# maniacs-ops/ringpop-go

Measured on AMD Instinct MI355X. Metric: simulated member-rounds/sec at 64k members, higher is better.
Workload: dtype u32; 1 GPU; config3_cascade: 65536 members, 655 killed at r=10; rounds 5-592 timed (steady state, kill, suspect wave; faulty wave from r>=35 in window); members=65536, live_member_rounds=38153303, parallelism=1 GPU

## Files before the change

### include/swimsim.h

```cpp
#ifndef SWIMSIM_H
#define SWIMSIM_H
#include <stddef.h>
#include <stdint.h>

#ifdef __cplusplus
extern "C" {
#endif

#define SWIMSIM_ABI_VERSION 16

enum {
    SWIMSIM_OK = 0,
    SWIMSIM_EINVAL = -1,
    SWIMSIM_ENOMEM = -2,
    SWIMSIM_EHIP = -3,
    SWIMSIM_ECAPACITY = -4,
    SWIMSIM_ERANGE = -5
};

enum { SWIMSIM_ALIVE = 0, SWIMSIM_SUSPECT = 1, SWIMSIM_FAULTY = 2, SWIMSIM_LEAVE = 3, SWIMSIM_TOMBSTONE = 4,
       SWIMSIM_UNKNOWN = 7 };
#define SWIMSIM_SOURCE_NONE (-1)

typedef struct swimsim_config {
    uint32_t num_members;
    uint32_t device;
    int64_t t0_ms;
    uint32_t protocol_period_ms;
    uint32_t suspect_timeout_ms;
    uint32_t faulty_timeout_ms;
    uint32_t tombstone_timeout_ms;
    uint32_t ping_request_size;
    uint32_t max_reverse_full_sync_jobs;
    uint32_t p_factor;
    uint64_t seed;
    const char *addresses;
    uint32_t addr_stride;
    uint32_t max_rounds;
    uint64_t message_pool_bytes;
    uint32_t observer_begin, observer_end;
    const struct swimsim_tuning *tuning;
} swimsim_config;

typedef struct swimsim_tuning {
    int32_t hot_slots;
    int32_t dense_slots;
    int32_t cs_async;
    int32_t cs_async_rows;
    int32_t cs_narrow_rows;
    int32_t cs_ref;
    int32_t fault_inject;
    int32_t defer_test;
    int32_t cs_defer;
    int32_t resp_echo;
} swimsim_tuning;

enum {
    SWIMSIM_EV_KILL = 1,
    SWIMSIM_EV_REVIVE = 2,
    SWIMSIM_EV_REINCARNATE = 3,
    SWIMSIM_EV_LEAVE = 4,
    SWIMSIM_EV_PARTITION = 5,
    SWIMSIM_EV_HEAL = 6,
    SWIMSIM_EV_REAP = 7,
    SWIMSIM_EV_CLOCK = 8
};
typedef struct swimsim_event { uint32_t round; uint32_t kind; int32_t a; int32_t b; } swimsim_event;

enum {
    SWIMSIM_C_ROUNDS, SWIMSIM_C_PINGS, SWIMSIM_C_PINGS_OK, SWIMSIM_C_PINGREQS, SWIMSIM_C_HELPER_CALLS,
    SWIMSIM_C_HELPER_ERRORS, SWIMSIM_C_INCONCLUSIVE, SWIMSIM_C_SUSPECT_DECL, SWIMSIM_C_APPLIED,
    SWIMSIM_C_REFUTES, SWIMSIM_C_FULL_SYNCS, SWIMSIM_C_FULL_SYNCS_PINGREQ, SWIMSIM_C_RFS_DONE,
    SWIMSIM_C_RFS_OMITTED, SWIMSIM_C_TIMERS_FIRED, SWIMSIM_C_MSG_CHANGES, SWIMSIM_C_HEAL_ATTEMPTS,
    SWIMSIM_C_HEAL_FAILURES, SWIMSIM_NCOUNTERS
};

typedef struct swimsim swimsim_t;
// ... 139 lines not shown
```

### ringpop-go_amd/csrc/swimsim_device.h

```cpp
#pragma once
#include <hip/hip_runtime.h>
#include <stdint.h>

namespace swimdev {

constexpr uint32_t ST_ALIVE = 0, ST_SUSPECT = 1, ST_FAULTY = 2, ST_LEAVE = 3, ST_TOMB = 4, ST_UNKNOWN = 7;
constexpr uint32_t SRC_NONE = 0xFFFFFFFFu;
constexpr uint32_t NO_DEADLINE = 0xFFFFFFFFu;
constexpr uint8_t DP_NONE = 0xFF;
constexpr uint32_t DE_NONE = 0xFFFFFFFFu;
__host__ __device__ inline uint32_t de_p(uint32_t x) { return x >> 24; }
__host__ __device__ inline uint32_t de_src(uint32_t x) { return (x & 0xFFFFFFu) == 0xFFFFFFu ? SRC_NONE : (x & 0xFFFFFFu); }
__host__ __device__ inline uint32_t de_x(uint32_t src, uint32_t p) { return (src & 0xFFFFFFu) | (p << 24); }

enum Counter {
    C_ROUNDS, C_PINGS, C_PINGS_OK, C_PINGREQS, C_HELPER_CALLS, C_HELPER_ERRORS, C_INCONCLUSIVE,
    C_SUSPECT_DECL, C_APPLIED, C_REFUTES, C_FULL_SYNCS, C_FULL_SYNCS_PINGREQ, C_RFS_DONE, C_RFS_OMITTED,
    C_TIMERS_FIRED, C_MSG_CHANGES, C_HEAL_ATTEMPTS, C_HEAL_FAILURES, C_NCOUNTERS,
    C_X_MERGED = C_NCOUNTERS, C_X_APPLIED, C_X_ISSUED, C_X_CS_ROWS, C_X_CS_DUP,
    C_X_MERGED_R, C_X_APPLIED_R, C_X_RISSUED, C_X_RCALLS, C_X_BUMPED, C_X_CS_ROWS_N, C_X_CSD_SCANNED,
    C_X_DENSE_RESP, C_X_DENSE_JOBS, C_X_JOBS_APPLIED, C_X_DENSE_HEAL,
    C_X_DEFER, C_X_DEFER_EQ, C_X_DEFER_NOROW, C_X_DEFER_REP, C_X_DEFER_UNDO,
    C_X_DEFER_REP_DIFF, C_X_DEFER_UNDO_DIFF, C_X_DEFER_FS, C_X_DEFER_UNDO_OVER, C_X_DEFER_CLEAN,
    C_X_ISSUE_SNAPS, C_X_LAZY_LATE, C_X_LAZY_MAT,
    C_X_ECHO, C_NALL
};

constexpr int CTR_SHARDS = 64, CTR_STRIDE = 64;
static_assert(C_NALL <= CTR_STRIDE, "counter block too small");
constexpr uint32_t POOL_SHARDS = 64, POOL_CUR_STRIDE = 16;

enum ErrBits : uint32_t {
    E_POOL = 1, E_DENSE = 2, E_ECAP = 4, E_SHORT = 8, E_ITER = 16, E_COUNT = 32, E_XCAP = 64
};

struct MsgDesc {
    uint32_t off_lo, off_hi;
    uint32_t len;
    uint32_t kind;
};

struct DS {
    uint32_t N, NP, NL, lo, NB, NBW;
    uint32_t W;
    uint32_t pfactor, K, maxjobs;
    uint32_t to_susp, to_faulty, to_tomb;
    uint32_t ecap;
    uint64_t seed;
// ... 42 lines not shown
    uint64_t wev_mask;
    uint4 **wevs;
    unsigned long long **wevts;
    uint32_t *wev_cnt;
    uint32_t wev_cap;
    unsigned long long *useq;
    uint32_t *hidx;
    uint32_t *hlist;
    uint32_t *hmw;
    uint2 *hde;
    uint32_t *colx;
    uint32_t *hotnew;
    uint32_t *hot_cnt;
    uint32_t HP;
    int32_t *nhe;
    uint32_t *ucl, *uhk, *ucold, *ucnt;
    uint2 *ulog;
    uint32_t *ulog_cnt;
    uint32_t ulog_cap;
    uint32_t ulog_stride;
    uint32_t defer_test;
    uint32_t *ilen;
    int32_t *ilast;
};
constexpr uint32_t ULOG_CAP = 1024, ULOG_STRIDE = ULOG_CAP + 256;
constexpr uint32_t SRC_PEND = 0x7FFFFFFEu, SRC_CLAIM = 0x7FFFFFFDu;
constexpr uint32_t DIRTY_CARRIED = 2u;

__device__ __forceinline__ uint32_t hot_slot(const DS &d, uint32_t m) { return d.hidx ? d.hidx[m] : SRC_NONE; }

__host__ __device__ inline bool is_pingable(uint32_t st) { return st <= ST_SUSPECT; }

__device__ __forceinline__ uint32_t clock_of(const DS &d, uint32_t o, uint32_t r) { return r + (uint32_t)d.coff[o]; }

constexpr uint32_t RT_LOOKUP = 0, RT_COLD = 8191, RT_MAXSLOTS = 8128;
__host__ __device__ inline uint32_t rec_m(const uint4 &r) { return r.x & 0xFFFFFFu; }
__host__ __device__ inline uint32_t rec_st(const uint4 &r) { return (r.x >> 24) & 7u; }
__host__ __device__ inline uint32_t rec_e(const uint4 &r) { return r.y & 0xFFFFFFu; }
__host__ __device__ inline uint32_t rec_tag(const uint4 &r) { return (r.x >> 27) | ((r.y >> 24) << 5); }
__host__ __device__ inline uint32_t tag_of_slot(uint32_t hk) { return hk == SRC_NONE ? RT_COLD : hk + 1u; }
__host__ __device__ inline uint4 rec_make(uint32_t m, uint32_t st, uint32_t e, uint32_t src, uint32_t sinc, uint32_t tag) {
    return make_uint4(m | (st << 24) | (tag << 27), e | ((tag >> 5) << 24), src, sinc);
}
__host__ __device__ inline uint4 rec_retag(const uint4 &r, uint32_t tag) {
    return make_uint4((r.x & 0x07FFFFFFu) | (tag << 27), (r.y & 0xFFFFFFu) | ((tag >> 5) << 24), r.z, r.w);
}
// ... 142 lines not shown
```

### ringpop-go_amd/csrc/swimsim_engine.hip

```cpp
#include "swimsim_kernels.hip"
#include "swimsim_xchg.hip"
#include "swimsim_census.hip"
#include "swimsim_route.hip"
#include "swimsim_forward.hip"
#include "swimsim_ringcs.hip"

#include <hipcub/hipcub.hpp>
#include <rccl/rccl.h>

#include <algorithm>
#include <cmath>
#include <condition_variable>
#include <cstdarg>
#include <cstdio>
#include <cstring>
#include <memory>
#include <mutex>
#include <string>
#include <thread>
#include <vector>

#include "../../include/swimsim.h"

using namespace swimdev;
// ... 340 lines not shown
    unsigned long long *rc_key = nullptr;
    uint32_t *rc_cnt = nullptr, *rc_rep = nullptr, *rc_dif = nullptr, *rc_hl = nullptr, *rc_csr = nullptr, *rc_out = nullptr;
    size_t rc_cap = 0;
    bool rc_lds = false;
    double rc_split[3] = {0, 0, 0};
    int32_t *fw_own = nullptr, *fw_handler = nullptr, *fw_holder = nullptr, *fw_next = nullptr;
    uint32_t *fw_ent = nullptr, *fw_key = nullptr, *fw_bins = nullptr;
    uint8_t *fw_outcome = nullptr, *fw_hops = nullptr;
    size_t fw_own_cap = 0, fw_req_cap = 0, fw_ent_cap = 0, fw_bins_cap = 0;
    double fw_split[3] = {0, 0, 0};
    int csr_mode = 1;
    CsrSet csr, csr2;
    size_t csr_sbw_words = 0;
    uint32_t csr_ecap = 4096, csr_rcap = 1024, csr_KP = 0;
    uint64_t csr_launches = 0;
    uint32_t csr_side_min = 4097;
    int fault_inject = 0;
    int defer_test = 0;
    int cs_defer = 1;
    uint32_t rounds_left = 0;
    uint32_t round_deferred = 0;
    bool cs_carried = false;
    int resp_echo = 1;
    bool cs_defer_log = false;
    uint64_t cs_skipped_rounds = 0, cs_carried_rows = 0, cs_forced = 0, cs_units_base[3] = {0, 0, 0};
    bool colx_stale = false;
    std::string err;

    int fail(int code, const char *fmt, ...) {
        char buf[512];
        va_list ap;
        va_start(ap, fmt);
        vsnprintf(buf, sizeof buf, fmt, ap);
        va_end(ap);
        err = buf;
        return code;
    }
};

#define HIPCHK(h, x)                                                                             \
    do {                                                                                         \
        hipError_t e_ = (x);                                                                     \
        if (e_ != hipSuccess) return (h)->fail(SWIMSIM_EHIP, "%s: %s", #x, hipGetErrorString(e_)); \
    } while (0)

namespace {
// ... 485 lines not shown
    if (st && nrows != ~0u && csr_side_wanted(h, n)) {
        if (h->csr2_used) HIPCHK(h, hipStreamWaitEvent(st, h->ev_csr2, 0));
        const int rc = csr_hash(h, h->csr2, list, cnt, n, st);
        HIPCHK(h, hipEventRecord(h->ev_csr2, st));
        h->csr2_used = true;
        if (rc <= 0) return rc;
    }
    Scope sc(h, kind == CS_WIDE ? F_CS_WIDE : F_CS_NARROW, st);
    launch_checksum_kind(h->d, list, cnt, n, kind, st ? st : h->s);
    return 0;
}

void hot_flush(swimsim *h, uint32_t ol0, uint32_t n) {
    if (!h->d.hidx || n == 0) return;
    hipLaunchKernelGGL(k_hot_flush, dim3(blocks_for_waves(n)), dim3(SWIM_WAVE_BLOCK), 0, h->s, h->d, ol0, n);
}

void hot_reset(swimsim *h, bool flush) {
    if (!h->d.hidx) return;
    if (flush) hot_flush(h, 0, h->NL);
    hipMemsetAsync(h->d.hidx, 0xFF, (size_t)h->N * 4, h->s);
    hipMemsetAsync(h->d.hotnew, 0, (size_t)h->d.NBIT * 4, h->s);
    hipMemsetAsync(h->d.hot_cnt, 0, 8, h->s);
    hipLaunchKernelGGL(k_nhe_reset, dim3(blocks_for_threads(h->NL)), dim3(256), 0, h->s, h->d);
}

void hot_update(swimsim *h) {
    if (!h->d.hidx) return;
    hipLaunchKernelGGL(k_hot_extend, dim3(1), dim3(1024), 0, h->s, h->d);
    hipLaunchKernelGGL(k_hot_fill, dim3(blocks_for_waves(h->NL)), dim3(SWIM_WAVE_BLOCK), 0, h->s, h->d);
}

int retire_half(swimsim *h, uint32_t g) {
    if (!h->side_pend[g]) return 0;
    HIPCHK(h, hipStreamWaitEvent(h->s, h->ev_side[g], 0));
    const uint32_t lo = h->d.dense_cap + g * h->snap_cap;
    hipLaunchKernelGGL(k_side_retire, dim3(blocks_for_threads(h->NL)), dim3(256), 0, h->s, h->d, lo, lo + h->snap_cap);
    h->side_pend[g] = false;
    h->side_pending = h->side_pend[0] || h->side_pend[1];
    return 0;
}

int sync_side(swimsim *h) {
    if (!h->side_pending) return 0;
    for (uint32_t g = 0; g < 2; g++)
        if (int rc = retire_half(h, (h->side_gen + g) % 2)) return rc;
// ... 704 lines not shown
        hipEventCreateWithFlags(&h->ev_side[0], hipEventDisableTiming) != hipSuccess ||
        hipEventCreateWithFlags(&h->ev_side[1], hipEventDisableTiming) != hipSuccess ||
        hipEventCreateWithFlags(&h->ev_rt, hipEventDisableTiming) != hipSuccess) {
        h->err = "hipStreamCreate / hipEventCreate failed";
        return bail(SWIMSIM_EHIP);
    }
    const swimsim_tuning *tun = cfg->tuning;
    if (tun && tun->cs_async >= 0) h->cs_async = tun->cs_async != 0;
    if (tun && tun->cs_narrow_rows >= 0) h->cs_narrow_rows = (uint32_t)tun->cs_narrow_rows;
    if (tun && tun->cs_ref >= 0) h->csr_mode = tun->cs_ref;
    if (tun && tun->fault_inject > 0) h->fault_inject = tun->fault_inject;
    if (tun && tun->defer_test > 0) h->defer_test = tun->defer_test;
    if (tun && tun->cs_defer >= 0) h->cs_defer = tun->cs_defer;
    if (const char *v = getenv("SWIMSIM_CS_DEFER")) h->cs_defer = atoi(v);
    if (const char *v = getenv("SWIMSIM_CS_DEFER_LOG")) h->cs_defer_log = atoi(v) != 0;
    if (h->cs_defer < 0 || h->cs_defer > 2) {
        h->err = "swimsim_tuning.cs_defer is -1, 0, 1 or 2";
        return bail(SWIMSIM_EINVAL);
    }
    if (tun && tun->resp_echo >= 0) h->resp_echo = tun->resp_echo;
    if (const char *v = getenv("SWIMSIM_RESP_ECHO")) h->resp_echo = atoi(v);
    if (h->resp_echo < 0 || h->resp_echo > 1) {
        h->err = "swimsim_tuning.resp_echo is -1, 0 or 1";
        return bail(SWIMSIM_EINVAL);
    }
    if (h->fault_inject & 32) h->csr_ecap = 24;
    if (h->fault_inject & 256) h->csr_side_min = 1024;
    if (const char *v = getenv("SWIMSIM_SYNC_SPIN")) h->sync_spin = atoi(v) != 0;
    if (const char *v = getenv("SWIMSIM_SIDE2"))
        if (atoi(v) == 0 && h->side2) { hipStreamDestroy(h->side2); h->side2 = nullptr; }
    DS &d = h->d;
    d.N = h->N; d.NP = h->NP; d.NL = h->NL; d.lo = h->lo;
    d.NB = h->NP / 64;
    d.NBW = (d.NB + 63) / 64;
    d.NBIT = ((h->NP / 32) + 3) & ~3u;
    d.W = h->W; d.pfactor = h->pfactor; d.K = h->K; d.maxjobs = h->maxjobs;
    d.to_susp = h->to_susp; d.to_faulty = h->to_faulty; d.to_tomb = h->to_tomb;
    d.seed = h->seed;
    const size_t rows = (size_t)h->NL * h->NP;
    int rc = 0;
    if ((rc = dalloc(h, &d.mw, rows, "member words")) || (rc = dalloc(h, &d.dent, rows, "dissemination entries")) ||
        (rc = dalloc(h, &d.tst, rows, "timer states")) ||
        (rc = dalloc(h, &d.tmr, rows, "timers")) ||
        (rc = dalloc(h, &d.ping, h->NL, "ping")) || (rc = dalloc(h, &d.maxp, h->NL, "maxp")) ||
        (rc = dalloc(h, &d.dcnt, h->NL, "dcnt")) || (rc = dalloc(h, &d.dirty, h->NL, "dirty")) ||
        (rc = dalloc(h, &d.cs, h->NL, "cs")) || (rc = dalloc(h, &d.it_idx, h->NL, "it_idx")) ||
        (rc = dalloc(h, &d.it_ep, h->NL, "it_ep")) || (rc = dalloc(h, &d.tmin, h->NL, "tmin")) ||
        (rc = dalloc(h, &d.njobs, h->NL, "njobs")) || (rc = dalloc(h, &d.jobs, (size_t)h->NL * h->maxjobs, "jobs")) ||
        (rc = dalloc(h, &d.dbit, (size_t)h->NL * d.NBIT, "dbit")) || (rc = dalloc(h, &d.tblk, (size_t)h->NL * d.NB, "tblk")) ||
        (rc = dalloc(h, &d.live, h->N, "live")) || (rc = dalloc(h, &d.part, h->N, "part")) ||
        (rc = dalloc(h, &d.coff, h->N, "clock offsets")) ||
        (rc = dalloc(h, &d.ctr, (size_t)CTR_SHARDS * CTR_STRIDE, "counters")) || (rc = dalloc(h, &d.err, 4, "err")) ||
        (rc = dalloc(h, &d.clen, h->NL, "clen")) || (rc = dalloc(h, &d.clast, h->NL, "clast")) ||
        (rc = dalloc(h, &d.cpslot, h->NL, "cpslot")) || (rc = dalloc(h, &d.nhe, h->NL, "cold entry counts")) ||
        (rc = dalloc(h, &d.colx, d.NBIT, "divergent columns")) || (rc = dalloc(h, &d.ucl, h->N, "divergent column list")) ||
        (rc = dalloc(h, &d.uhk, h->N, "divergent column hot slots")) || (rc = dalloc(h, &d.ucold, h->N, "cold divergent columns")) ||
        (rc = dalloc(h, &d.ucnt, 2, "divergent column counts")))
        return bail(rc);
    hipMemset(d.nhe, 0, (size_t)h->NL * 4);
    hipMemset(d.coff, 0, (size_t)h->N * 4);
    h->coff.assign(h->N, 0);
    hipMemset(d.colx, 0xFF, (size_t)d.NBIT * 4);
    hipMemset(d.cpslot, 0xFF, (size_t)h->NL * 4);
    {
        uint32_t hp = std::min<uint32_t>(2048u, h->NP);
        if (tun && tun->hot_slots >= 0) hp = std::min<uint32_t>((uint32_t)tun->hot_slots, h->NP);
        hp = std::min<uint32_t>((hp + 63) & ~63u, RT_MAXSLOTS);
        d.hidx = nullptr; d.hlist = nullptr; d.hmw = nullptr; d.hde = nullptr; d.hotnew = nullptr; d.hot_cnt = nullptr;
        d.HP = 0;
        if (hp) {
            if ((rc = dalloc(h, &d.hidx, h->N, "hot index")) || (rc = dalloc(h, &d.hlist, hp, "hot list")) ||
                (rc = dalloc(h, &d.hmw, (size_t)h->NL * hp, "hot member words")) ||
                (rc = dalloc(h, &d.hde, (size_t)h->NL * hp, "hot dissemination cells")) ||
                (rc = dalloc(h, &d.hotnew, d.NBIT, "hot candidates")) || (rc = dalloc(h, &d.hot_cnt, 2, "hot count")))
                return bail(rc);
            d.HP = hp;
            hot_reset(h, false);
        }
    }
    {
        std::vector<uint32_t> aw((size_t)h->N * 6, 0u);
        for (uint32_t m = 0; m < h->N; m++) {
            uint8_t b[24] = {0};
            memcpy(b, h->addrs[m].data(), h->W);
            for (int w = 0; w < 6; w++)
                aw[(size_t)m * 6 + w] = (uint32_t)b[4 * w] | ((uint32_t)b[4 * w + 1] << 8) | ((uint32_t)b[4 * w + 2] << 16) |
                                        ((uint32_t)b[4 * w + 3] << 24);
        }
        uint32_t *dev = nullptr;
        if ((rc = dalloc(h, &dev, aw.size(), "address words"))) return bail(rc);
        if (hipMemcpy(dev, aw.data(), aw.size() * 4, hipMemcpyHostToDevice) != hipSuccess) return bail(SWIMSIM_EHIP);
        d.addrw = dev;
// ... 1071 lines not shown
            if (f == F_CSPREP) b = csdups * 8.0 * h->N;
            if (f == F_CSD_SCAN) b = delta(C_X_CSD_SCANNED) * 4.0 * h->N;
            if (f == F_ISSUE) b = issued * 32.0;
            if (f == F_RECV) b = merge_bytes + recv_issue_bytes;
            if (f == F_RESP) b = resp_bytes;
            if (f == F_JOBS_MERGE) b = delta(C_X_DENSE_JOBS) * 5.0 * h->N + delta(C_X_JOBS_APPLIED) * 23.0;
            alg_bytes[f] = b;
        }
    }
    if (n) *n = F_NFAM;
    return SWIMSIM_OK;
}

int swimsim_kernel_units(swimsim_t *h, const char **names, double *values, size_t cap, size_t *n) {
    if (!h) return SWIMSIM_EINVAL;
    uint64_t c[CTR_STRIDE];
    if (int rc = read_counters(h, c)) return rc;
    static const char *kn[] = {"cs_rows_wide", "cs_rows_narrow", "cs_dup_rows", "recv_merged", "recv_applied",
                               "recv_issued", "recv_calls", "resp_merged", "resp_applied", "resp_bumped", "issued",
                               "bitmap_words_per_row", "hot_slots", "dense_resp", "dense_jobs", "jobs_applied",
                               "dense_heal", "defer", "defer_eq", "defer_norow", "defer_rep", "defer_undo",
                               "defer_rep_diff", "defer_undo_diff", "defer_fs", "defer_undo_over", "defer_clean",
                               "issue_snaps", "lazy_late", "lazy_mat", "resp_echoed",
                               "cs_skipped_rounds", "cs_carried_rows", "cs_forced"};
    const int ki[] = {C_X_CS_ROWS, C_X_CS_ROWS_N, C_X_CS_DUP, C_X_MERGED, C_X_APPLIED, C_X_RISSUED, C_X_RCALLS,
                      C_X_MERGED_R, C_X_APPLIED_R, C_X_BUMPED, C_X_ISSUED, -1, -2, C_X_DENSE_RESP, C_X_DENSE_JOBS,
                      C_X_JOBS_APPLIED, C_X_DENSE_HEAL, C_X_DEFER, C_X_DEFER_EQ, C_X_DEFER_NOROW, C_X_DEFER_REP,
                      C_X_DEFER_UNDO, C_X_DEFER_REP_DIFF, C_X_DEFER_UNDO_DIFF, C_X_DEFER_FS, C_X_DEFER_UNDO_OVER,
                      C_X_DEFER_CLEAN, C_X_ISSUE_SNAPS, C_X_LAZY_LATE, C_X_LAZY_MAT, C_X_ECHO,
                      -3, -4, -5};
    const uint64_t lazy_c[3] = {h->cs_skipped_rounds - h->cs_units_base[0], h->cs_carried_rows - h->cs_units_base[1],
                                h->cs_forced - h->cs_units_base[2]};
    static_assert(sizeof(kn) / sizeof(kn[0]) == sizeof(ki) / sizeof(ki[0]), "one counter per name");
    uint32_t hot = 0;
    if (h->d.hot_cnt) {
        HIPCHK(h, hipMemcpyAsync(&hot, h->d.hot_cnt, 4, hipMemcpyDeviceToHost, h->s));
        HIPCHK(h, stream_sync(h));
    }
    const size_t k = sizeof(ki) / sizeof(ki[0]);
    for (size_t i = 0; i < k && i < cap; i++) {
        if (names) names[i] = kn[i];
        if (values)
            values[i] = ki[i] == -1 ? (double)h->d.NBIT : ki[i] == -2 ? (double)hot : ki[i] <= -3 ? (double)lazy_c[-3 - ki[i]]
                                                                                : (double)(c[ki[i]] - h->fam_bytes_base[ki[i]]);
    }
    if (n) *n = k;
    return SWIMSIM_OK;
}

int swimsim_group_create(const swimsim_config *cfg, uint32_t nshards, const int32_t *devices, swimsim_t **out) {
    if (!cfg || !out || nshards < 1 || nshards > 64 || cfg->num_members < nshards) return SWIMSIM_EINVAL;
    const std::vector<uint32_t> lo = canonical_split(cfg->num_members, nshards);
    auto hub = std::make_shared<LocalHub>(nshards);
// ... 188 lines not shown
```

### ringpop-go_amd/csrc/swimsim_kernels.hip

```cpp
#include "swimsim_kernels.h"

namespace swimdev {

#define SWIM_DPP(old, src, ctrl, rm) ((uint32_t)__builtin_amdgcn_update_dpp((int)(old), (int)(src), (ctrl), (rm), 0xf, false))
template <typename Op>
__device__ __forceinline__ uint32_t dpp_scan(uint32_t x, uint32_t id, Op op) {
    x = op(x, SWIM_DPP(id, x, 0x111, 0xf));
    x = op(x, SWIM_DPP(id, x, 0x112, 0xf));
    x = op(x, SWIM_DPP(id, x, 0x114, 0xf));
    x = op(x, SWIM_DPP(id, x, 0x118, 0xf));
    x = op(x, SWIM_DPP(id, x, 0x142, 0xa));
    x = op(x, SWIM_DPP(id, x, 0x143, 0xc));
    return x;
}
__device__ __forceinline__ uint32_t dpp_scan_add(uint32_t x) { return dpp_scan(x, 0u, [](uint32_t a, uint32_t b) { return a + b; }); }
__device__ __forceinline__ uint32_t dpp_scan_umin(uint32_t x) {
    return dpp_scan(x, 0xFFFFFFFFu, [](uint32_t a, uint32_t b) { return min(a, b); });
}
__device__ __forceinline__ int32_t dpp_scan_imax(int32_t x) {
    return (int32_t)dpp_scan((uint32_t)x, 0x80000000u, [](uint32_t a, uint32_t b) { return (uint32_t)max((int32_t)a, (int32_t)b); });
}
__device__ __forceinline__ int32_t dpp_scan_imin(int32_t x) {
    return (int32_t)dpp_scan((uint32_t)x, 0x7FFFFFFFu, [](uint32_t a, uint32_t b) { return (uint32_t)min((int32_t)a, (int32_t)b); });
}
// ... 444 lines not shown
                nx = x[u] + (1u << 24);
            }
            if (hk[u] != SRC_NONE) hx[(size_t)hk[u] * 2] = nx;
            else dx[(size_t)m[u] * 2] = nx;
        }
    }
    return make_int2(wsum(del), wsum(delnh));
}
__device__ void wave_bump(const DS &d, uint32_t ol, const MsgDesc &md) {
    if (md.kind != 0) return;
    const int2 dd = wave_bump_body(d, ol, md, d.maxp[ol]);
    if (lane_id() == 0 && dd.x) d.dcnt[ol] -= dd.x;
    if (lane_id() == 0 && dd.y) d.nhe[ol] -= dd.y;
    __threadfence_block();
}
__device__ __forceinline__ void wave_bump_pre(const DS &d, uint32_t ol, const MsgDesc &md, RowPre &p) {
    if (md.kind != 0) return;
    const int2 dd = wave_bump_body(d, ol, md, p.maxp);
    if (dd.x) { p.dcnt -= dd.x; if (lane_id() == 0) d.dcnt[ol] = p.dcnt; }
    if (dd.y) { p.nhe -= dd.y; if (lane_id() == 0) d.nhe[ol] = p.nhe; }
    __threadfence_block();
}

__device__ __forceinline__ unsigned long long pool_alloc_lane0(const DS &d, uint32_t n) {
    const unsigned long long sub = d.pool_cap / POOL_SHARDS;
    const bool small = n <= sub / 256;
    for (uint32_t t = 0, s = wave_gid() % POOL_SHARDS; t < POOL_SHARDS; t++, s = (s + 1) % POOL_SHARDS) {
        unsigned long long *cur = d.pool_cur + (size_t)s * POOL_CUR_STRIDE;
        if (small) {
            const unsigned long long old = atomicAdd(cur, (unsigned long long)n);
            if (old + n <= sub) return s * sub + old;
            continue;
        }
        unsigned long long old = __hip_atomic_load(cur, __ATOMIC_RELAXED, __HIP_MEMORY_SCOPE_AGENT);
        while (old + n <= sub) {
            const unsigned long long seen = atomicCAS(cur, old, old + n);
            if (seen == old) return s * sub + old;
            old = seen;
        }
    }
    atomicOr(d.err, E_POOL);
    return ~0ull;
}
__device__ __forceinline__ unsigned long long pool_alloc(const DS &d, uint32_t n) {
    unsigned long long off = 0;
    if (lane_id() == 0 && n) off = pool_alloc_lane0(d, n);
    return bcast64(off);
}

__device__ __forceinline__ uint32_t wscan_excl(uint32_t v, uint32_t &total) {
    const uint32_t x = dpp_scan_add(v);
    total = lane63(x);
    return x - v;
}

template <bool RECV>
__device__ __forceinline__ uint32_t wave_issue_body(const DS &d, uint32_t ol, uint32_t sender, uint32_t sinc, MsgDesc &out,
                                                    uint32_t cnt, int maxp, bool hotwalk, uint32_t nslots,
                                                    unsigned long long off, int &del_out, int &delnh_out,
                                                    const uint32_t *echo = nullptr) {
    const size_t rb = (size_t)ol * d.NP, hb = (size_t)ol * d.HP;
    uint32_t *bits = d.dbit + (size_t)ol * d.NBIT;
    uint32_t pos = 0;
    uint32_t kept = 0;
    int del = 0, delnh = 0;
    const bool skip = RECV && echo != nullptr;
    auto echo_word = [&](uint32_t hk) { return skip && hk != SRC_NONE ? echo[hk >> 5] : 0u; };
    if (hotwalk) {
        for (uint32_t base = 0; base < nslots; base += 64 * MB) {
            uint2 ce[MB];
            uint32_t wv[MB], m[MB], ew[MB];
#pragma unroll
            for (int u = 0; u < MB; u++) {
                const uint32_t k = base + u * 64 + lane_id();
                ce[u] = k < nslots ? d.hde[hb + k] : make_uint2(DE_NONE, 0);
                wv[u] = k < nslots ? d.hmw[hb + k] : 0u;
                m[u] = k < nslots ? d.hlist[k] : 0u;
                ew[u] = echo_word(k < nslots ? k : SRC_NONE);
            }
            bool keep[MB], wr[MB];
            uint32_t nk = 0;
#pragma unroll
            for (int u = 0; u < MB; u++) {
                const uint32_t src = de_src(ce[u].x);
                keep[u] = de_p(ce[u].x) != DP_NONE && !(RECV && src == sender && ce[u].y == sinc);
                wr[u] = keep[u] && !((ew[u] >> (lane_id() & 31)) & 1u);
                kept += keep[u] ? 1u : 0u;
                nk += wr[u] ? 1u : 0u;
            }
            uint32_t tot;
            uint32_t at = pos + wscan_excl(nk, tot);
#pragma unroll
            for (int u = 0; u < MB; u++) {
                if (!keep[u]) continue;
                const uint32_t st = (wv[u] & 7u) == ST_UNKNOWN ? ST_TOMB : (wv[u] & 7u);
                if (wr[u]) {
                    if (at < cnt) d.pool[off + at] = rec_make(m[u], st, wv[u] >> 3, de_src(ce[u].x), ce[u].y, base + u * 64 + lane_id() + 1u);
                    at++;
                }
                if (RECV) {
                    const uint32_t k = base + u * 64 + lane_id();
                    uint32_t nx;
                    if ((int)(de_p(ce[u].x) + 1) >= maxp) {
                        nx = ce[u].x | 0xFF000000u;
                        atomicAnd(bits + (m[u] >> 5), ~(1u << (m[u] & 31)));
                        del++;
                    } else {
                        nx = ce[u].x + (1u << 24);
                    }
                    d.hde[hb + k].x = nx;
                }
            }
            pos += tot;
        }
// ... 150 lines not shown
            }
            pos += tot;
        }
        if (RECV && (dlo | dhi)) {
            if (dlo & 0xFFFFFFFFull) atomicAnd(bits + q + 0, ~(uint32_t)dlo);
            if (dlo >> 32) atomicAnd(bits + q + 1, ~(uint32_t)(dlo >> 32));
            if (dhi & 0xFFFFFFFFull) atomicAnd(bits + q + 2, ~(uint32_t)dhi);
            if (dhi >> 32) atomicAnd(bits + q + 3, ~(uint32_t)(dhi >> 32));
        }
    }
    if (RECV) {
        del_out = wsum(del);
        delnh_out = wsum(delnh);
    } else if (pos != cnt && lane_id() == 0) {
        atomicOr(d.err, E_COUNT);
    }
    out.off_lo = (uint32_t)off;
    out.off_hi = (uint32_t)(off >> 32);
    out.len = min(pos, cnt);
    return skip ? min((uint32_t)wsum((int)kept), cnt) : out.len;
}

template <bool RECV>
__device__ uint32_t wave_issue_t(const DS &d, uint32_t ol, uint32_t sender, uint32_t sinc, MsgDesc &out) {
    const uint32_t cnt = (uint32_t)d.dcnt[ol];
    const int maxp = RECV ? d.maxp[ol] : 0;
    const bool hotwalk = d.hidx && d.nhe[ol] == 0;
    const uint32_t nslots = d.hidx ? d.hot_cnt[0] : 0u;
    out.kind = 0; out.len = 0; out.off_lo = out.off_hi = 0;
    if (cnt == 0) return 0;
    const unsigned long long off = pool_alloc(d, cnt);
    if (off == ~0ull) return 0;
    int del = 0, delnh = 0;
    const uint32_t n = wave_issue_body<RECV>(d, ol, sender, sinc, out, cnt, maxp, hotwalk, nslots, off, del, delnh);
    if (RECV) {
        if (lane_id() == 0 && del) d.dcnt[ol] -= del;
        if (lane_id() == 0 && delnh) d.nhe[ol] -= delnh;
    }
    __threadfence_block();
    return n;
}

__device__ void wave_issue(const DS &d, uint32_t ol, MsgDesc &out) { wave_issue_t<false>(d, ol, 0, 0, out); }

__device__ uint32_t wave_issue_recv(const DS &d, uint32_t ol, uint32_t sender, uint32_t sinc, MsgDesc &out) {
    return wave_issue_t<true>(d, ol, sender, sinc, out);
}

__device__ bool wave_snapshot(const DS &d, uint32_t ol, uint32_t o, MsgDesc &out) {
    uint32_t slot = 0;
    if (lane_id() == 0) slot = atomicAdd(d.dense_cur, 1u);
    slot = (uint32_t)__builtin_amdgcn_readlane((int)slot, 0);
    out.kind = 2; out.len = 0; out.off_lo = out.off_hi = 0;
    if (slot >= d.dense_cap) {
        if (lane_id() == 0) atomicOr(d.err, E_DENSE);
        return false;
    }
    const uint4 *src = (const uint4 *)(d.mw + (size_t)ol * d.NP);
    uint4 *dst = (uint4 *)(d.dense + (size_t)slot * d.NP);
    int known = 0;
    const uint32_t n4 = d.NP / 4;
    for (uint32_t i = lane_id(); i < n4; i += 64 * SNAP_MB) {
        uint4 v[SNAP_MB];
#pragma unroll
        for (int u = 0; u < SNAP_MB; u++) v[u] = i + u * 64 < n4 ? src[i + u * 64] : make_uint4(ST_UNKNOWN, ST_UNKNOWN, ST_UNKNOWN, ST_UNKNOWN);
#pragma unroll
// ... 382 lines not shown

__global__ void k_carry(DS d) {
    const uint32_t ol = blockIdx.x * blockDim.x + threadIdx.x;
    if (ol < d.NL && d.dirty[ol]) d.dirty[ol] = DIRTY_CARRIED;
}

__global__ void k_list_one(uint32_t *list, uint32_t *cnt, uint32_t ol, const DS d) {
    if (threadIdx.x == 0) { *cnt = d.dirty[ol] ? 1u : 0u; list[0] = ol; }
}

__global__ void k_issue(DS d, int mode, const int32_t *tgt, const uint8_t *failed, MsgDesc *sdesc, uint32_t *sI,
                        uint32_t *sC, uint32_t *sS) {
    const uint32_t ol = wave_gid();
    if (ol >= d.NL) return;
    const uint32_t o = d.lo + ol;
    if ((mode == 0 && tgt[ol] < 0) || (mode == 1 && !failed[ol])) {
        if (sS && lane_id() == 0) sS[o] = SRC_NONE;
        return;
    }
    const uint32_t dirty = d.dirty[ol], cpslot = d.cpslot[ol], cs = d.cs[ol], selfw = d.mw[(size_t)ol * d.NP + o];
    const uint32_t clen = d.clen[ol];
    const int32_t clast = d.clast[ol];
    MsgDesc md;
    wave_issue(d, ol, md);
    uint32_t slot = SRC_NONE;
    if (sS && dirty && !d.ulog) {
        MsgDesc sn;
        if (wave_snapshot(d, ol, o, sn)) slot = sn.off_lo;
        if (lane_id() == 0) ctr_add(d, C_X_ISSUE_SNAPS, 1ull);
    } else if (sS && dirty) {
        slot = SRC_PEND;
        if (lane_id() == 0) { d.ilen[ol] = clen; d.ilast[ol] = clast; }
    } else if (sS) {
        slot = cpslot;
    }
    if (lane_id() == 0) {
        sdesc[o] = md;
        sI[o] = selfw >> 3;
        sC[o] = slot == SRC_NONE ? cs : 0u;
        if (sS) sS[o] = slot;
        if (mode == 0) {
            ctr_add(d, C_PINGS, 1ull);
            ctr_add(d, C_MSG_CHANGES, (unsigned long long)md.len);
        }
        ctr_add(d, C_X_ISSUED, (unsigned long long)md.len);
    }
}
// ... 596 lines not shown

__global__ void k_build_jobs(DS d, const uint32_t *counts, const uint32_t *offs, const uint32_t *vals,
                             uint8_t *fsflag) {
    const uint32_t u = blockIdx.x * blockDim.x + threadIdx.x, ol = u;
    if (u >= d.NL) return;
    for (uint32_t w = 0; w < counts[u]; w++) {
        const uint32_t p = offs[u] + w;
        if (!fsflag[p]) continue;
        fsflag[p] = 0;
        if (d.njobs[ol] < d.maxjobs) d.jobs[(size_t)ol * d.maxjobs + d.njobs[ol]++] = vals[p];
        else ctr_add(d, C_RFS_OMITTED, 1ull);
    }
}

__global__ void k_resp(DS d, const int32_t *tgt, const uint8_t *failed, const MsgDesc *sdesc, const MsgDesc *rdesc,
                       uint32_t r) {
    const uint32_t ol = wave_gid();
    if (ol >= d.NL) return;
    if (tgt[ol] < 0 || failed[ol]) return;
    const uint32_t o = d.lo + ol;
    RowPre p = row_pre(d, ol);
    const uint32_t now = wave_clock(d, o, r);
    const MsgDesc sd = sdesc[o], rd = rdesc[o];
    uint4 rec0[MB];
    merge_first(d, rd, rec0);
    wave_bump_pre(d, ol, sd, p);
    if (rd.kind != 0 || rd.len)
        wave_merge_msg_pre(d, ol, o, rd, now, now, 1, p, C_X_DENSE_RESP, rec0);
    if (lane_id() == 0) {
        ctr_add(d, C_PINGS_OK, 1ull);
        if (sd.kind == 0) ctr_add(d, C_X_BUMPED, (unsigned long long)sd.len);
    }
}

__global__ void k_resolve(DS d, const int32_t *tgt, const uint8_t *failed, const uint32_t *H, const uint32_t *nh,
                          const MsgDesc *sdesc2, const MsgDesc *rdesc2, uint32_t r) {
    const uint32_t ol = wave_gid();
    if (ol >= d.NL || !failed[ol]) return;
    const uint32_t o = d.lo + ol, K = d.K;
    const uint32_t now = wave_clock(d, o, r);
    uint32_t errs = 0;
    for (uint32_t q = 0; q < nh[ol]; q++) {
        const uint32_t h = H[(size_t)ol * K + q];
        if (!reach(d, o, h)) {
            errs++;
            wave_bump(d, ol, sdesc2[o]);
        } else {
            const MsgDesc rd = rdesc2[(size_t)o * K + q];
            if (rd.kind != 0 || rd.len) wave_merge_msg(d, ol, o, rd, now, now, 2, C_X_DENSE_RESP);
        }
    }
    if (lane_id() == 0) {
        if (errs) ctr_add(d, C_HELPER_ERRORS, (unsigned long long)errs);
        if (errs == K) {
            ctr_add(d, C_INCONCLUSIVE, 1ull);
        } else {
            ctr_add(d, C_SUSPECT_DECL, 1ull);
            const uint32_t t = (uint32_t)tgt[ol];
            const uint32_t te = d.mw[(size_t)ol * d.NP + t] >> 3;
            thread_make_change(d, ol, o, t, te, ST_SUSPECT, now);
        }
    }
}

__global__ void k_jobs_mark(DS d, uint8_t *need) {
    const uint32_t ol = blockIdx.x * blockDim.x + threadIdx.x;
    if (ol >= d.NL) return;
    for (uint32_t q = 0; q < d.njobs[ol]; q++) need[d.jobs[(size_t)ol * d.maxjobs + q]] = 1;
}
// ... 365 lines not shown
```

### ringpop-go_amd/swimsim/__init__.py

```python
from __future__ import annotations

import ctypes as C
import os
from dataclasses import dataclass

import numpy as np

_HERE = os.path.dirname(os.path.abspath(__file__))
LIB_PATH = os.path.join(_HERE, "libswimsim.so")

ALIVE, SUSPECT, FAULTY, LEAVE, TOMBSTONE, UNKNOWN = 0, 1, 2, 3, 4, 7
STATUS_NAMES = {ALIVE: "alive", SUSPECT: "suspect", FAULTY: "faulty", LEAVE: "leave", TOMBSTONE: "tombstone"}
SOURCE_NONE = -1
EV_KILL, EV_REVIVE, EV_REINCARNATE, EV_LEAVE, EV_PARTITION, EV_HEAL, EV_REAP = 1, 2, 3, 4, 5, 6, 7
EV_CLOCK = 8
COUNTER_NAMES = [
    "rounds", "pings", "pings_ok", "pingreqs", "helper_calls", "helper_errors", "inconclusive",
    "suspect_decl", "applied", "refutes", "full_syncs", "full_syncs_pingreq", "rfs_done",
    "rfs_omitted", "timers_fired", "msg_changes", "heal_attempts", "heal_failures",
]
T0_MS = 1_500_000_000_000
CENSUS_LIVE, CENSUS_ALL = 0, 1
CENSUS_WHO = {"live": CENSUS_LIVE, "all": CENSUS_ALL}
ROUTE_N_REPLICAS = 16
# ... 8 lines not shown
ERRORS = {-1: "EINVAL", -2: "ENOMEM", -3: "EHIP", -4: "ECAPACITY", -5: "ERANGE"}


class SwimsimError(RuntimeError):
    pass


class Config(C.Structure):
    _fields_ = [
        ("num_members", C.c_uint32), ("device", C.c_uint32), ("t0_ms", C.c_int64),
        ("protocol_period_ms", C.c_uint32), ("suspect_timeout_ms", C.c_uint32), ("faulty_timeout_ms", C.c_uint32),
        ("tombstone_timeout_ms", C.c_uint32), ("ping_request_size", C.c_uint32),
        ("max_reverse_full_sync_jobs", C.c_uint32), ("p_factor", C.c_uint32), ("seed", C.c_uint64),
        ("addresses", C.c_char_p), ("addr_stride", C.c_uint32), ("max_rounds", C.c_uint32),
        ("message_pool_bytes", C.c_uint64), ("observer_begin", C.c_uint32), ("observer_end", C.c_uint32),
        ("tuning", C.c_void_p),
    ]


class Tuning(C.Structure):
    _fields_ = [("hot_slots", C.c_int32), ("dense_slots", C.c_int32), ("cs_async", C.c_int32),
                ("cs_async_rows", C.c_int32), ("cs_narrow_rows", C.c_int32), ("cs_ref", C.c_int32),
                ("fault_inject", C.c_int32), ("defer_test", C.c_int32), ("cs_defer", C.c_int32),
                ("resp_echo", C.c_int32)]


def make_tuning(tuning):
    if not tuning:
        return None
    t = Tuning(*([-1] * len(Tuning._fields_)))
    for k, v in tuning.items():
        if k not in dict(Tuning._fields_):
            raise ValueError(f"unknown tuning field {k}")
        setattr(t, k, int(v))
    return t


class Event(C.Structure):
    _fields_ = [("round", C.c_uint32), ("kind", C.c_uint32), ("a", C.c_int32), ("b", C.c_int32)]


_U64P = C.POINTER(C.c_uint64)
ALLTOALL_U64 = C.CFUNCTYPE(C.c_int, C.c_void_p, _U64P, _U64P, C.c_int32)
ALLTOALLV = C.CFUNCTYPE(C.c_int, C.c_void_p, C.c_void_p, _U64P, _U64P, C.c_void_p, _U64P, _U64P)
BCAST = C.CFUNCTYPE(C.c_int, C.c_void_p, C.c_void_p, C.c_size_t, C.c_uint32)


# ... 1167 lines not shown
```

Measured before the change: 124.8 million member-rounds/s.

## Record sent hot-slot bitmaps at issue and bump piggyback counts by slot

When a member issues a ping message from the hot-slot walk, a per-row bitmap now records which hot slots were included, plus a validity count. On a failed ping or ping-req, the piggyback-count bump walks that bitmap over the hot dissemination entries instead of re-parsing the sent message from the pool. This avoids decoding records from the message pool on the bump path. In exchange it adds bitmap writes to every issue and extra memory per row, and it depends on the bitmap staying consistent with the slot layout, with a fallback to the old path when it is not valid.

```diff
diff --git a/include/swimsim.h b/include/swimsim.h
--- a/include/swimsim.h
+++ b/include/swimsim.h
@@ -7,7 +7,7 @@
 extern "C" {
 #endif
 
-#define SWIMSIM_ABI_VERSION 16
+#define SWIMSIM_ABI_VERSION 17
 
 enum {
     SWIMSIM_OK = 0,
@@ -53,6 +53,7 @@
     int32_t defer_test;
     int32_t cs_defer;
     int32_t resp_echo;
+    int32_t slot_bump;
 } swimsim_tuning;
 
 enum {
diff --git a/ringpop-go_amd/csrc/swimsim_device.h b/ringpop-go_amd/csrc/swimsim_device.h
--- a/ringpop-go_amd/csrc/swimsim_device.h
+++ b/ringpop-go_amd/csrc/swimsim_device.h
@@ -23,7 +23,8 @@
     C_X_DEFER, C_X_DEFER_EQ, C_X_DEFER_NOROW, C_X_DEFER_REP, C_X_DEFER_UNDO,
     C_X_DEFER_REP_DIFF, C_X_DEFER_UNDO_DIFF, C_X_DEFER_FS, C_X_DEFER_UNDO_OVER, C_X_DEFER_CLEAN,
     C_X_ISSUE_SNAPS, C_X_LAZY_LATE, C_X_LAZY_MAT,
-    C_X_ECHO, C_NALL
+    C_X_ECHO,
+    C_X_BUMP_SLOT, C_NALL
 };
 
 constexpr int CTR_SHARDS = 64, CTR_STRIDE = 64;
@@ -112,6 +113,8 @@
     uint32_t defer_test;
     uint32_t *ilen;
     int32_t *ilast;
+    unsigned long long *sbm;
+    uint32_t *sbv;
 };
 constexpr uint32_t ULOG_CAP = 1024, ULOG_STRIDE = ULOG_CAP + 256;
 constexpr uint32_t SRC_PEND = 0x7FFFFFFEu, SRC_CLAIM = 0x7FFFFFFDu;
diff --git a/ringpop-go_amd/csrc/swimsim_engine.hip b/ringpop-go_amd/csrc/swimsim_engine.hip
--- a/ringpop-go_amd/csrc/swimsim_engine.hip
+++ b/ringpop-go_amd/csrc/swimsim_engine.hip
@@ -386,6 +386,7 @@
     uint32_t round_deferred = 0;
     bool cs_carried = false;
     int resp_echo = 1;
+    int slot_bump = 1;
     bool cs_defer_log = false;
     uint64_t cs_skipped_rounds = 0, cs_carried_rows = 0, cs_forced = 0, cs_units_base[3] = {0, 0, 0};
     bool colx_stale = false;
@@ -917,6 +918,7 @@
     hipMemsetAsync(h->d.hidx, 0xFF, (size_t)h->N * 4, h->s);
     hipMemsetAsync(h->d.hotnew, 0, (size_t)h->d.NBIT * 4, h->s);
     hipMemsetAsync(h->d.hot_cnt, 0, 8, h->s);
+    if (h->d.sbv) hipMemsetAsync(h->d.sbv, 0, (size_t)h->NL * 4, h->s);
     hipLaunchKernelGGL(k_nhe_reset, dim3(blocks_for_threads(h->NL)), dim3(256), 0, h->s, h->d);
 }
 
@@ -1667,6 +1669,12 @@
     if (const char *v = getenv("SWIMSIM_RESP_ECHO")) h->resp_echo = atoi(v);
     if (h->resp_echo < 0 || h->resp_echo > 1) {
         h->err = "swimsim_tuning.resp_echo is -1, 0 or 1";
+        return bail(SWIMSIM_EINVAL);
+    }
+    if (tun && tun->slot_bump >= 0) h->slot_bump = tun->slot_bump;
+    if (const char *v = getenv("SWIMSIM_SLOT_BUMP")) h->slot_bump = atoi(v);
+    if (h->slot_bump < 0 || h->slot_bump > 1) {
+        h->err = "swimsim_tuning.slot_bump is -1, 0 or 1";
         return bail(SWIMSIM_EINVAL);
     }
     if (h->fault_inject & 32) h->csr_ecap = 24;
@@ -1713,6 +1721,12 @@
         hp = std::min<uint32_t>((hp + 63) & ~63u, RT_MAXSLOTS);
         d.hidx = nullptr; d.hlist = nullptr; d.hmw = nullptr; d.hde = nullptr; d.hotnew = nullptr; d.hot_cnt = nullptr;
         d.HP = 0;
+        d.sbm = nullptr; d.sbv = nullptr;
+        if (hp && h->slot_bump) {
+            if ((rc = dalloc(h, &d.sbm, (size_t)h->NL * (hp / 64), "sent-slot bitmaps")) ||
+                (rc = dalloc(h, &d.sbv, h->NL, "sent-slot bitmap validity")))
+                return bail(rc);
+        }
         if (hp) {
             if ((rc = dalloc(h, &d.hidx, h->N, "hot index")) || (rc = dalloc(h, &d.hlist, hp, "hot list")) ||
                 (rc = dalloc(h, &d.hmw, (size_t)h->NL * hp, "hot member words")) ||
@@ -2830,13 +2844,13 @@
                                "dense_heal", "defer", "defer_eq", "defer_norow", "defer_rep", "defer_undo",
                                "defer_rep_diff", "defer_undo_diff", "defer_fs", "defer_undo_over", "defer_clean",
                                "issue_snaps", "lazy_late", "lazy_mat", "resp_echoed",
-                               "cs_skipped_rounds", "cs_carried_rows", "cs_forced"};
+                               "cs_skipped_rounds", "cs_carried_rows", "cs_forced", "bump_by_slot"};
     const int ki[] = {C_X_CS_ROWS, C_X_CS_ROWS_N, C_X_CS_DUP, C_X_MERGED, C_X_APPLIED, C_X_RISSUED, C_X_RCALLS,
                       C_X_MERGED_R, C_X_APPLIED_R, C_X_BUMPED, C_X_ISSUED, -1, -2, C_X_DENSE_RESP, C_X_DENSE_JOBS,
                       C_X_JOBS_APPLIED, C_X_DENSE_HEAL, C_X_DEFER, C_X_DEFER_EQ, C_X_DEFER_NOROW, C_X_DEFER_REP,
                       C_X_DEFER_UNDO, C_X_DEFER_REP_DIFF, C_X_DEFER_UNDO_DIFF, C_X_DEFER_FS, C_X_DEFER_UNDO_OVER,
                       C_X_DEFER_CLEAN, C_X_ISSUE_SNAPS, C_X_LAZY_LATE, C_X_LAZY_MAT, C_X_ECHO,
-                      -3, -4, -5};
+                      -3, -4, -5, C_X_BUMP_SLOT};
     const uint64_t lazy_c[3] = {h->cs_skipped_rounds - h->cs_units_base[0], h->cs_carried_rows - h->cs_units_base[1],
                                 h->cs_forced - h->cs_units_base[2]};
     static_assert(sizeof(kn) / sizeof(kn[0]) == sizeof(ki) / sizeof(ki[0]), "one counter per name");
diff --git a/ringpop-go_amd/csrc/swimsim_kernels.hip b/ringpop-go_amd/csrc/swimsim_kernels.hip
--- a/ringpop-go_amd/csrc/swimsim_kernels.hip
+++ b/ringpop-go_amd/csrc/swimsim_kernels.hip
@@ -490,6 +490,58 @@
     __threadfence_block();
 }
 
+constexpr int SB_U = 12;
+__device__ __forceinline__ int wave_bump_slots(const DS &d, uint32_t ol, uint32_t nslots, int maxp) {
+    uint32_t *hx = (uint32_t *)(d.hde + (size_t)ol * d.HP);
+    const unsigned long long *bm = d.sbm + (size_t)ol * (d.HP / 64);
+    int del = 0;
+    for (uint32_t base = 0; base < nslots; base += 64 * SB_U) {
+        uint32_t x[SB_U], m[SB_U];
+        const uint32_t g = (base >> 6) + lane_id();
+        const unsigned long long wl = lane_id() < (uint32_t)SB_U && g * 64 < nslots ? bm[g] : 0ull;
+#pragma unroll
+        for (int u = 0; u < SB_U; u++) {
+            const uint32_t k = base + u * 64 + lane_id();
+            x[u] = k < nslots ? hx[(size_t)k * 2] : DE_NONE;
+            m[u] = k < nslots ? d.hlist[k] : 0u;
+        }
+#pragma unroll
+        for (int u = 0; u < SB_U; u++) {
+            const uint32_t k = base + u * 64 + lane_id();
+            const uint32_t p = de_p(x[u]);
+            const uint32_t wlo = (uint32_t)__builtin_amdgcn_readlane((int)(uint32_t)wl, u);
+            const uint32_t whi = (uint32_t)__builtin_amdgcn_readlane((int)(uint32_t)(wl >> 32), u);
+            const uint32_t wh = lane_id() < 32 ? wlo : whi;
+            if (!((wh >> (lane_id() & 31)) & 1u) || p == DP_NONE) continue;
+            uint32_t nx;
+            if ((int)(p + 1) >= maxp) {
+                nx = x[u] | 0xFF000000u;
+                atomicAnd(&d.dbit[(size_t)ol * d.NBIT + (m[u] >> 5)], ~(1u << (m[u] & 31)));
+                del++;
+            } else {
+                nx = x[u] + (1u << 24);
+            }
+            hx[(size_t)k * 2] = nx;
+        }
+    }
+    return wsum(del);
+}
+__device__ __forceinline__ bool bump_by_slot(const MsgDesc &md, uint32_t sbn) { return sbn && md.kind == 0 && md.len; }
+__device__ void wave_bump_slot(const DS &d, uint32_t ol, uint32_t nslots) {
+    const int del = wave_bump_slots(d, ol, nslots, d.maxp[ol]);
+    if (lane_id() == 0) {
+        if (del) d.dcnt[ol] -= del;
+        ctr_add(d, C_X_BUMP_SLOT, 1ull);
+    }
+    __threadfence_block();
+}
+__device__ __forceinline__ void wave_bump_slot_pre(const DS &d, uint32_t ol, uint32_t nslots, RowPre &p) {
+    const int del = wave_bump_slots(d, ol, nslots, p.maxp);
+    if (del) { p.dcnt -= del; if (lane_id() == 0) d.dcnt[ol] = p.dcnt; }
+    if (lane_id() == 0) ctr_add(d, C_X_BUMP_SLOT, 1ull);
+    __threadfence_block();
+}
+
 __device__ __forceinline__ unsigned long long pool_alloc_lane0(const DS &d, uint32_t n) {
     const unsigned long long sub = d.pool_cap / POOL_SHARDS;
     const bool small = n <= sub / 256;
@@ -526,7 +578,7 @@
 __device__ __forceinline__ uint32_t wave_issue_body(const DS &d, uint32_t ol, uint32_t sender, uint32_t sinc, MsgDesc &out,
                                                     uint32_t cnt, int maxp, bool hotwalk, uint32_t nslots,
                                                     unsigned long long off, int &del_out, int &delnh_out,
-                                                    const uint32_t *echo = nullptr) {
+                                                    const uint32_t *echo = nullptr, unsigned long long *sent = nullptr) {
     const size_t rb = (size_t)ol * d.NP, hb = (size_t)ol * d.HP;
     uint32_t *bits = d.dbit + (size_t)ol * d.NBIT;
     uint32_t pos = 0;
@@ -558,6 +610,15 @@
             }
             uint32_t tot;
             uint32_t at = pos + wscan_excl(nk, tot);
+            if (!RECV && sent) {
+                unsigned long long kb = 0;
+#pragma unroll
+                for (int u = 0; u < MB; u++) {
+                    const unsigned long long b = __ballot(keep[u]);
+                    if (lane_id() == (uint32_t)u) kb = b;
+                }
+                if (lane_id() < (uint32_t)MB && base + lane_id() * 64 < nslots) sent[(base >> 6) + lane_id()] = kb;
+            }
 #pragma unroll
             for (int u = 0; u < MB; u++) {
                 if (!keep[u]) continue;
@@ -754,17 +815,23 @@
 }
 
 template <bool RECV>
-__device__ uint32_t wave_issue_t(const DS &d, uint32_t ol, uint32_t sender, uint32_t sinc, MsgDesc &out) {
+__device__ uint32_t wave_issue_t(const DS &d, uint32_t ol, uint32_t sender, uint32_t sinc, MsgDesc &out, bool mark = false) {
     const uint32_t cnt = (uint32_t)d.dcnt[ol];
     const int maxp = RECV ? d.maxp[ol] : 0;
     const bool hotwalk = d.hidx && d.nhe[ol] == 0;
     const uint32_t nslots = d.hidx ? d.hot_cnt[0] : 0u;
+    mark = mark && !RECV && d.sbm;
     out.kind = 0; out.len = 0; out.off_lo = out.off_hi = 0;
-    if (cnt == 0) return 0;
-    const unsigned long long off = pool_alloc(d, cnt);
-    if (off == ~0ull) return 0;
+    const unsigned long long off = cnt ? pool_alloc(d, cnt) : ~0ull;
+    if (off == ~0ull) {
+        if (mark && lane_id() == 0) d.sbv[ol] = 0u;
+        return 0;
+    }
     int del = 0, delnh = 0;
-    const uint32_t n = wave_issue_body<RECV>(d, ol, sender, sinc, out, cnt, maxp, hotwalk, nslots, off, del, delnh);
+    unsigned long long *sent = mark && hotwalk ? d.sbm + (size_t)ol * (d.HP / 64) : nullptr;
+    const uint32_t n = wave_issue_body<RECV>(d, ol, sender, sinc, out, cnt, maxp, hotwalk, nslots, off, del, delnh, nullptr,
+                                             sent);
+    if (mark && lane_id() == 0) d.sbv[ol] = sent && out.len == cnt ? nslots : 0u;
     if (RECV) {
         if (lane_id() == 0 && del) d.dcnt[ol] -= del;
         if (lane_id() == 0 && delnh) d.nhe[ol] -= delnh;
@@ -773,7 +840,9 @@
     return n;
 }
 
-__device__ void wave_issue(const DS &d, uint32_t ol, MsgDesc &out) { wave_issue_t<false>(d, ol, 0, 0, out); }
+__device__ void wave_issue(const DS &d, uint32_t ol, MsgDesc &out, bool mark = false) {
+    wave_issue_t<false>(d, ol, 0, 0, out, mark);
+}
 
 __device__ uint32_t wave_issue_recv(const DS &d, uint32_t ol, uint32_t sender, uint32_t sinc, MsgDesc &out) {
     return wave_issue_t<true>(d, ol, sender, sinc, out);
@@ -1202,7 +1271,7 @@
     const uint32_t clen = d.clen[ol];
     const int32_t clast = d.clast[ol];
     MsgDesc md;
-    wave_issue(d, ol, md);
+    wave_issue(d, ol, md, true);
     uint32_t slot = SRC_NONE;
     if (sS && dirty && !d.ulog) {
         MsgDesc sn;
@@ -1845,9 +1914,11 @@
     RowPre p = row_pre(d, ol);
     const uint32_t now = wave_clock(d, o, r);
     const MsgDesc sd = sdesc[o], rd = rdesc[o];
+    const uint32_t sbn = d.sbv ? uni(d.sbv[ol]) : 0u;
     uint4 rec0[MB];
     merge_first(d, rd, rec0);
-    wave_bump_pre(d, ol, sd, p);
+    if (bump_by_slot(sd, sbn)) wave_bump_slot_pre(d, ol, sbn, p);
+    else wave_bump_pre(d, ol, sd, p);
     if (rd.kind != 0 || rd.len)
         wave_merge_msg_pre(d, ol, o, rd, now, now, 1, p, C_X_DENSE_RESP, rec0);
     if (lane_id() == 0) {
@@ -1863,11 +1934,14 @@
     const uint32_t o = d.lo + ol, K = d.K;
     const uint32_t now = wave_clock(d, o, r);
     uint32_t errs = 0;
+    const MsgDesc sd = sdesc2[o];
+    const uint32_t sbn = d.sbv ? uni(d.sbv[ol]) : 0u;
     for (uint32_t q = 0; q < nh[ol]; q++) {
         const uint32_t h = H[(size_t)ol * K + q];
         if (!reach(d, o, h)) {
             errs++;
-            wave_bump(d, ol, sdesc2[o]);
+            if (bump_by_slot(sd, sbn)) wave_bump_slot(d, ol, sbn);
+            else wave_bump(d, ol, sd);
         } else {
             const MsgDesc rd = rdesc2[(size_t)o * K + q];
             if (rd.kind != 0 || rd.len) wave_merge_msg(d, ol, o, rd, now, now, 2, C_X_DENSE_RESP);
diff --git a/ringpop-go_amd/swimsim/__init__.py b/ringpop-go_amd/swimsim/__init__.py
--- a/ringpop-go_amd/swimsim/__init__.py
+++ b/ringpop-go_amd/swimsim/__init__.py
@@ -54,7 +54,7 @@
     _fields_ = [("hot_slots", C.c_int32), ("dense_slots", C.c_int32), ("cs_async", C.c_int32),
                 ("cs_async_rows", C.c_int32), ("cs_narrow_rows", C.c_int32), ("cs_ref", C.c_int32),
                 ("fault_inject", C.c_int32), ("defer_test", C.c_int32), ("cs_defer", C.c_int32),
-                ("resp_echo", C.c_int32)]
+                ("resp_echo", C.c_int32), ("slot_bump", C.c_int32)]
 
 
 def make_tuning(tuning):
```

Result: faster. 127.5 million member-rounds/s (median of 6 runs) (+2.1%).
